# LinXueyuanStdio/LaTeX_OCR

Measured on NVIDIA H100. Metric: formula-images/sec (train step, 128x512 px, seq<=150), higher is better.
Workload: dtype bf16

## Files before the change

### latex_ocr_b200/csrc/lo_tc.cu

```cuda
#include <cuda.h>

#include <mutex>
#include <unordered_map>

#include "lo_common.cuh"
#include "lo_ptx.cuh"
#include "lo_wgmma.cuh"

namespace lo {

__device__ __forceinline__ void tma_load_2d(void* dst, const CUtensorMap* map, uint64_t* bar, int c0, int c1) {
  asm volatile("cp.async.bulk.tensor.2d.shared::cluster.global.mbarrier::complete_tx::bytes [%0], [%1, {%3, %4}], [%2];" ::"r"(
                   smem_u32(dst)),
               "l"(reinterpret_cast<uint64_t>(map)), "r"(smem_u32(bar)), "r"(c0), "r"(c1)
               : "memory");
}
__device__ __forceinline__ void tma_load_2d_hint(void* dst, const CUtensorMap* map, uint64_t* bar, int c0, int c1, uint64_t policy) {
  asm volatile(
      "cp.async.bulk.tensor.2d.shared::cluster.global.mbarrier::complete_tx::bytes.L2::cache_hint [%0], [%1, {%3, %4}], [%2], %5;" ::"r"(
          smem_u32(dst)),
      "l"(reinterpret_cast<uint64_t>(map)), "r"(smem_u32(bar)), "r"(c0), "r"(c1), "l"(policy)
      : "memory");
}
__device__ __forceinline__ void tma_load_3d(void* dst, const CUtensorMap* map, uint64_t* bar, int c0, int c1, int c2) {
// ... 62 lines not shown
  int64_t ldc;
  int out_f32, accumulate, relu;
  int kb_per_split, atomic;
  int w_evict_last;
  int half_w, half_h;
  long long* dbg;
  int lstm;
  const float* l_ptab; const int64_t* l_tok; int64_t l_tok_stride;
  const float* l_hh; int64_t l_hh_stride;
  const float* l_cprev; float* l_gates; float* l_c; float* l_h; bf16* l_hbf;
  float* l_hd; int64_t l_hd_stride; const float* l_dmask;
  int l_D, l_V;
};

constexpr int TC_BM = 128, TC_BK = 64;
constexpr int TC_CWARPS = 8;
constexpr int TC_THREADS = (TC_CWARPS + 2) * 32;

template <int NT, int STAGES>
struct TcSmem {
  static constexpr int A_BYTES = TC_BM * TC_BK * 2;
  static constexpr int B_BYTES = NT * TC_BK * 2;
  static constexpr int STAGE_BYTES = A_BYTES + B_BYTES;
  static constexpr int TOTAL = STAGES * STAGE_BYTES + 1024  + 256 ;
};

template <int NT>
__device__ __forceinline__ void tc_mma_kblock(float* acc, uint32_t sa, uint32_t sb, bool first) {
  const uint64_t da = make_kmajor_sw128_desc(sa), db = make_kmajor_sw128_desc(sb);
#pragma unroll
  for (int k = 0; k < TC_BK / 16; k++)
    Wgmma<NT, 0, 0>::mma(acc, da + (uint64_t)(2 * k), db + (uint64_t)(2 * k), (first && k == 0) ? 0u : 1u);
}

__device__ __forceinline__ void tc_store_pair(const TcParams& p, int64_t off, float f0, float f1, bool use_mask) {
  if (p.atomic) {
    float* o = reinterpret_cast<float*>(p.out) + off;
    atomicAdd(o, f0);
    atomicAdd(o + 1, f1);
  } else if (p.out_f32) {
    float2* o = reinterpret_cast<float2*>(reinterpret_cast<float*>(p.out) + off);
    if (p.accumulate) { const float2 old = *o; f0 += old.x; f1 += old.y; }
    if (p.relu) { f0 = fmaxf(f0, 0.f); f1 = fmaxf(f1, 0.f); }
    *o = make_float2(f0, f1);
  } else {
    uint32_t* o = reinterpret_cast<uint32_t*>(reinterpret_cast<bf16*>(p.out) + off);
    if (p.accumulate) { const uint32_t old = *o; f0 += __uint_as_float(old << 16); f1 += __uint_as_float(old & 0xffff0000u); }
    if (p.relu) { f0 = fmaxf(f0, 0.f); f1 = fmaxf(f1, 0.f); }
    if (use_mask) {
      const uint32_t w = *reinterpret_cast<const uint32_t*>(p.mask + off);
      if (!(__uint_as_float(w << 16) > 0.f)) f0 = 0.f;
      if (!(__uint_as_float(w & 0xffff0000u) > 0.f)) f1 = 0.f;
    }
    __nv_bfloat162 h = __floats2bfloat162_rn(f0, f1);
    *o = *reinterpret_cast<uint32_t*>(&h);
  }
}

template <int NT, int STAGES, int MC>
__global__ void __launch_bounds__(TC_THREADS, 1) tc_gemm_conv_kernel(const __grid_constant__ CUtensorMap mapA,
                                                                      const __grid_constant__ CUtensorMap mapB, TcParams p) {
  using SM = TcSmem<NT, STAGES>;
  extern __shared__ uint8_t smem_raw[];
  uint8_t* smem = reinterpret_cast<uint8_t*>((reinterpret_cast<uintptr_t>(smem_raw) + 1023) & ~(uintptr_t)1023);
  uint64_t* full_bar = reinterpret_cast<uint64_t*>(smem + STAGES * SM::STAGE_BYTES);
  uint64_t* empty_bar = full_bar + STAGES;
  __shared__ __align__(16) float s_bias[NT];

  const int warp = threadIdx.x >> 5, lane = threadIdx.x & 31;
  const int n0 = blockIdx.x * NT;
  const int mt = blockIdx.y;
  const int KB_all = p.K / TC_BK;
  const int kb0 = blockIdx.z * p.kb_per_split;
  const int KB = min(KB_all, kb0 + p.kb_per_split) - kb0;

  int img = 0, h0 = 0, w0 = 0, m0 = mt * TC_BM;
  if (p.conv) {
    const int per_img = p.tiles_w * p.tiles_h;
    img = mt / per_img;
    const int rem = mt % per_img;
    h0 = (rem / p.tiles_w) * p.BH;
    w0 = (rem % p.tiles_w) * p.BW;
  }

  const bool dbg = p.dbg && blockIdx.x == 0 && blockIdx.y == 0 && blockIdx.z == 0;
  if (dbg && threadIdx.x == 0) p.dbg[0] = clock64();
  if (warp == TC_CWARPS && lane == 0) {
    tma_prefetch_desc(&mapA);
    tma_prefetch_desc(&mapB);
    for (int s = 0; s < STAGES; s++) {
      mbar_init(full_bar + s, 2);
      mbar_init(empty_bar + s, MC ? 2 * TC_CWARPS : TC_CWARPS);
    }
    fence_barrier_init();
  }
  pdl_wait();
  pdl_trigger();
  if (MC) cluster_sync_all(); else __syncthreads();
  const uint32_t crank = MC ? cluster_ctarank() : 0;
  if (dbg && threadIdx.x == 0) p.dbg[1] = clock64();

  if (warp == TC_CWARPS) {
    if (lane == 0) {
      const int cpb = p.conv ? p.Cin / TC_BK : 1;
      for (int kb = 0; kb < KB; kb++) {
        const int s = kb % STAGES;
        const uint32_t ph = (kb / STAGES) & 1;
        mbar_wait(empty_bar + s, ph ^ 1);
        uint8_t* sa = smem + s * SM::STAGE_BYTES;
        mbar_expect_tx(full_bar + s, SM::A_BYTES);
        const int kg = kb0 + kb;
        if (MC) {
          uint8_t* sh = sa + crank * (SM::A_BYTES / 2);
          if (p.conv) {
            const int tap = kg / cpb, cb = kg % cpb;
            const int r = tap / 3, q = tap % 3;
            tma_load_4d_mc(sh, &mapA, full_bar + s, cb * TC_BK, w0 + (int)crank * p.half_w + q - p.pad,
                           h0 + (int)crank * p.half_h + r - p.pad, img, (uint16_t)3);
          } else {
            tma_load_2d_mc(sh, &mapA, full_bar + s, kg * TC_BK, m0 + (int)crank * (TC_BM / 2), (uint16_t)3);
          }
        } else if (p.conv) {
          const int tap = kg / cpb, cb = kg % cpb;
          const int r = tap / 3, q = tap % 3;
          tma_load_4d(sa, &mapA, full_bar + s, cb * TC_BK, w0 + q - p.pad, h0 + r - p.pad, img);
        } else {
          tma_load_2d(sa, &mapA, full_bar + s, kg * TC_BK, m0);
        }
        if (dbg && kb == 0) p.dbg[2] = clock64();
        if (dbg && kb < 40) p.dbg[64 + kb] = clock64();
      }
      if (dbg) p.dbg[3] = clock64();
    }
    __syncwarp();
  } else if (warp == TC_CWARPS + 1) {
    if (lane == 0) {
      const uint64_t polB = p.w_evict_last ? l2_policy_evict_last() : l2_policy_evict_normal();
      for (int kb = 0; kb < KB; kb++) {
        const int s = kb % STAGES;
        const uint32_t ph = (kb / STAGES) & 1;
        mbar_wait(empty_bar + s, ph ^ 1);
        uint8_t* sb = smem + s * SM::STAGE_BYTES + SM::A_BYTES;
        mbar_expect_tx(full_bar + s, SM::B_BYTES);
        tma_load_2d_hint(sb, &mapB, full_bar + s, (kb0 + kb) * TC_BK, n0, polB);
      }
    }
    __syncwarp();
  } else {
    const int wg = warp >> 2;
    for (int c = threadIdx.x; c < NT; c += TC_CWARPS * 32)
      s_bias[c] = (p.bias && blockIdx.z == 0 && n0 + c < p.N) ? __ldg(p.bias + n0 + c) : 0.f;
    asm volatile("bar.sync 1, 256;" ::: "memory");
    float acc[NT / 2];
    for (int kb = 0; kb < KB; kb++) {
      const int s = kb % STAGES;
      const uint32_t ph = (kb / STAGES) & 1;
      mbar_wait(full_bar + s, ph);
      if (dbg && threadIdx.x == 0 && kb == 0) p.dbg[4] = clock64();
      if (dbg && threadIdx.x == 0 && kb < 40) p.dbg[16 + kb] = clock64();
      const uint32_t sa = smem_u32(smem + s * SM::STAGE_BYTES);
      wgmma_fence();
      tc_mma_kblock<NT>(acc, sa + wg * (SM::A_BYTES / 2), sa + SM::A_BYTES, kb == 0);
      wgmma_commit();
      wgmma_wait0();
      wgmma_acc_fence<NT / 2>(acc);
      __syncwarp();
      if (lane == 0) {
        if (MC) { mbar_arrive_cta(empty_bar + s, 0); mbar_arrive_cta(empty_bar + s, 1); }
        else mbar_arrive(empty_bar + s);
      }
    }
    if (dbg && threadIdx.x == 0) p.dbg[5] = clock64();
    const int rbase = wg * 64 + (warp & 3) * 16 + (lane >> 2);
    const int cq = 2 * (lane & 3);
    if (p.lstm) {
      const int D = p.l_D;
#pragma unroll
      for (int h = 0; h < 2; h++) {
        const int b = m0 + rbase + 8 * h;
#pragma unroll
        for (int i = 0; i < NT / 8; i++) {
          const float a0 = acc[4 * i + 2 * h], a1 = acc[4 * i + 2 * h + 1];
          const float o0 = __shfl_xor_sync(0xffffffffu, a0, 1), o1 = __shfl_xor_sync(0xffffffffu, a1, 1);
          const int j = (n0 + 8 * i + cq) / 4;
          if ((lane & 1) || b >= p.M || j >= D) continue;
          int64_t tk = p.l_tok[(int64_t)b * p.l_tok_stride];
          tk = tk < 0 ? 0 : (tk >= p.l_V ? p.l_V - 1 : tk);
          const float* pt = p.l_ptab + tk * 4 * D;
          const float* hh = p.l_hh + (int64_t)b * p.l_hh_stride;
          const float pi = a0 + pt[j] + hh[j];
          const float pf = a1 + pt[D + j] + hh[D + j];
          const float pg = o0 + pt[2 * D + j] + hh[2 * D + j];
          const float po = o1 + pt[3 * D + j] + hh[3 * D + j];
          const float ig = sigmoidf_(pi), fg = sigmoidf_(pf), gg = tanhf(pg), og = sigmoidf_(po);
          const float cn = fg * p.l_cprev[(int64_t)b * D + j] + ig * gg;
          const float hn = og * tanhf(cn);
          float* gt = p.l_gates + (int64_t)b * 4 * D;
          gt[j] = ig; gt[D + j] = fg; gt[2 * D + j] = gg; gt[3 * D + j] = og;
          p.l_c[(int64_t)b * D + j] = cn;
          p.l_h[(int64_t)b * D + j] = hn;
          if (p.l_hbf) p.l_hbf[(int64_t)b * D + j] = __float2bfloat16_rn(hn);
          if (p.l_hd) p.l_hd[(int64_t)b * p.l_hd_stride + j] = p.l_dmask ? hn * p.l_dmask[(int64_t)b * p.l_hd_stride + j] : hn;
        }
      }
    } else {
      const bool use_mask = p.mask && !p.out_f32 && !p.atomic;
#pragma unroll
      for (int h = 0; h < 2; h++) {
        const int row = rbase + 8 * h;
        bool row_ok;
        int64_t row_off;
        if (p.conv) {
          const int hh = h0 + row / p.BW, ww = w0 + row % p.BW;
          row_ok = (hh < p.Ho) && (ww < p.Wo);
          row_off = (((int64_t)img * p.Ho + hh) * p.Wo + ww) * p.ldc;
        } else {
          row_ok = (m0 + row) < p.M;
          row_off = (int64_t)(m0 + row) * p.ldc;
        }
        if (!row_ok) continue;
#pragma unroll
        for (int i = 0; i < NT / 8; i++) {
          if (n0 + 8 * i >= p.N) continue;
          const int c = 8 * i + cq;
          tc_store_pair(p, row_off + n0 + c, acc[4 * i + 2 * h] + s_bias[c], acc[4 * i + 2 * h + 1] + s_bias[c + 1], use_mask);
        }
      }
    }
    if (dbg && threadIdx.x == 0) p.dbg[6] = clock64();
  }
  if (MC) cluster_sync_all();
  if (dbg && threadIdx.x == 0) p.dbg[7] = clock64();
}

template <int NT, int STAGES, int MT>
struct TcPSmem {
  static constexpr int A_BYTES = TC_BM * TC_BK * 2;
  static constexpr int B_BYTES = NT * TC_BK * 2;
  static constexpr int STAGE_BYTES = MT * A_BYTES + B_BYTES;
  static constexpr int TOTAL = STAGES * STAGE_BYTES + 1024  + 256  + 2 * NT * 4 ;
};

template <int NT, int STAGES, int MT>
__global__ void __launch_bounds__(TC_THREADS, 1) tc_conv_p_kernel(const __grid_constant__ CUtensorMap mapA,
                                                                 const __grid_constant__ CUtensorMap mapB, TcParams p, int ntiles_n,
                                                                 int total_tiles, int mtiles) {
  using SM = TcPSmem<NT, STAGES, MT>;
  static_assert(MT * NT <= 256, "accumulator registers");
  extern __shared__ uint8_t smem_raw[];
  uint8_t* smem = reinterpret_cast<uint8_t*>((reinterpret_cast<uintptr_t>(smem_raw) + 1023) & ~(uintptr_t)1023);
  uint64_t* full_bar = reinterpret_cast<uint64_t*>(smem + STAGES * SM::STAGE_BYTES);
  uint64_t* empty_bar = full_bar + STAGES;
  float* s_bias = reinterpret_cast<float*>(smem + STAGES * SM::STAGE_BYTES + 256);

  const int warp = threadIdx.x >> 5, lane = threadIdx.x & 31;
  const int KB = p.K / TC_BK;
  const int cpb = p.Cin / TC_BK;
  const int per_img = p.tiles_w * p.tiles_h;

  if (warp == TC_CWARPS && lane == 0) {
    tma_prefetch_desc(&mapA);
    tma_prefetch_desc(&mapB);
    for (int s = 0; s < STAGES; s++) {
      mbar_init(full_bar + s, 2);
      mbar_init(empty_bar + s, TC_CWARPS);
    }
    fence_barrier_init();
  }
  pdl_wait();
  pdl_trigger();
  __syncthreads();

  if (warp == TC_CWARPS) {
    if (lane == 0) {
      uint32_t it = 0;
      for (int tile = blockIdx.x; tile < total_tiles; tile += gridDim.x) {
        const int mt0 = (tile / ntiles_n) * MT;
        const int nsub = min(MT, mtiles - mt0);
        int img[MT], h0[MT], w0[MT];
#pragma unroll
        for (int j = 0; j < MT; j++) {
          const int mt = min(mt0 + j, mtiles - 1);
          img[j] = mt / per_img;
          const int rem = mt % per_img;
          h0[j] = (rem / p.tiles_w) * p.BH;
          w0[j] = (rem % p.tiles_w) * p.BW;
        }
        for (int kb = 0; kb < KB; kb++, it++) {
          const int s = it % STAGES;
          const uint32_t ph = (it / STAGES) & 1;
          mbar_wait(empty_bar + s, ph ^ 1);
          mbar_expect_tx(full_bar + s, (uint32_t)nsub * SM::A_BYTES);
          const int tap = kb / cpb, cb = kb % cpb;
          const int r = tap / 3, q = tap % 3;
#pragma unroll
          for (int j = 0; j < MT; j++)
            if (j < nsub)
              tma_load_4d(smem + s * SM::STAGE_BYTES + j * SM::A_BYTES, &mapA, full_bar + s, cb * TC_BK, w0[j] + q - p.pad,
                          h0[j] + r - p.pad, img[j]);
        }
      }
    }
    __syncwarp();
  } else if (warp == TC_CWARPS + 1) {
    if (lane == 0) {
      const uint64_t polB = l2_policy_evict_last();
      uint32_t it = 0;
      for (int tile = blockIdx.x; tile < total_tiles; tile += gridDim.x) {
        const int n0 = (tile % ntiles_n) * NT;
        for (int kb = 0; kb < KB; kb++, it++) {
          const int s = it % STAGES;
          const uint32_t ph = (it / STAGES) & 1;
          mbar_wait(empty_bar + s, ph ^ 1);
          mbar_expect_tx(full_bar + s, SM::B_BYTES);
          tma_load_2d_hint(smem + s * SM::STAGE_BYTES + MT * SM::A_BYTES, &mapB, full_bar + s, kb * TC_BK, n0, polB);
        }
      }
    }
    __syncwarp();
  } else {
    const int wg = warp >> 2;
    const int rbase = wg * 64 + (warp & 3) * 16 + (lane >> 2);
    const int cq = 2 * (lane & 3);
    const bool use_mask = p.mask != nullptr;
    uint32_t it = 0, lt = 0;
    for (int tile = blockIdx.x; tile < total_tiles; tile += gridDim.x, lt++) {
      const int n0 = (tile % ntiles_n) * NT;
      const int mt0 = (tile / ntiles_n) * MT;
      const int nsub = min(MT, mtiles - mt0);
      float* sb = s_bias + (lt & 1) * NT;
      for (int c = threadIdx.x; c < NT; c += TC_CWARPS * 32) sb[c] = (p.bias && n0 + c < p.N) ? __ldg(p.bias + n0 + c) : 0.f;
      asm volatile("bar.sync 1, 256;" ::: "memory");
      float acc[MT][NT / 2];
      for (int kb = 0; kb < KB; kb++, it++) {
        const int s = it % STAGES;
        const uint32_t ph = (it / STAGES) & 1;
        mbar_wait(full_bar + s, ph);
        const uint32_t sa = smem_u32(smem + s * SM::STAGE_BYTES);
        wgmma_fence();
#pragma unroll
        for (int j = 0; j < MT; j++)
          tc_mma_kblock<NT>(acc[j], sa + j * SM::A_BYTES + wg * (SM::A_BYTES / 2), sa + MT * SM::A_BYTES, kb == 0);
        wgmma_commit();
        wgmma_wait0();
#pragma unroll
        for (int j = 0; j < MT; j++) wgmma_acc_fence<NT / 2>(acc[j]);
        __syncwarp();
        if (lane == 0) mbar_arrive(empty_bar + s);
      }
#pragma unroll
      for (int j = 0; j < MT; j++) {
        if (j >= nsub) continue;
        const int mt = mt0 + j;
        const int img = mt / per_img, rem = mt % per_img;
#pragma unroll
        for (int h = 0; h < 2; h++) {
          const int row = rbase + 8 * h;
          const int hh = (rem / p.tiles_w) * p.BH + row / p.BW, ww = (rem % p.tiles_w) * p.BW + row % p.BW;
          if (hh >= p.Ho || ww >= p.Wo) continue;
          const int64_t row_off = (((int64_t)img * p.Ho + hh) * p.Wo + ww) * p.ldc;
#pragma unroll
          for (int i = 0; i < NT / 8; i++) {
            if (n0 + 8 * i >= p.N) continue;
            const int c = 8 * i + cq;
            float f0 = acc[j][4 * i + 2 * h] + sb[c], f1 = acc[j][4 * i + 2 * h + 1] + sb[c + 1];
            if (p.relu) { f0 = fmaxf(f0, 0.f); f1 = fmaxf(f1, 0.f); }
            if (use_mask) {
              const uint32_t w = *reinterpret_cast<const uint32_t*>(p.mask + row_off + n0 + c);
              if (!(__uint_as_float(w << 16) > 0.f)) f0 = 0.f;
              if (!(__uint_as_float(w & 0xffff0000u) > 0.f)) f1 = 0.f;
            }
            __nv_bfloat162 hv = __floats2bfloat162_rn(f0, f1);
            *reinterpret_cast<__nv_bfloat162*>(reinterpret_cast<bf16*>(p.out) + row_off + n0 + c) = hv;
          }
        }
      }
    }
  }
}

__device__ __forceinline__ uint64_t make_mnmajor_sw128_desc(uint32_t saddr, uint32_t lbo_bytes) {
  uint64_t d = 0;
  d |= (uint64_t)((saddr & 0x3FFFF) >> 4);
  d |= (uint64_t)((lbo_bytes >> 4) & 0x3FFF) << 16;
  d |= (uint64_t)(1024 >> 4) << 32;
  d |= (uint64_t)1 << 62;
  return d;
}

struct WgParams {
  int Cin, Cout, Ho, Wo, pad;
  int BW, BH, tiles_w, tiles_h, kstages, per_split, ci_tiles;
  float* dw;
  int plain;
  int64_t ldc;
  int64_t batch_c;
  int ordered;
};

template <int NT, int STAGES>
__global__ void __launch_bounds__(TC_THREADS, 1) tc_wgrad_kernel(const __grid_constant__ CUtensorMap mapDY,
                                                                  const __grid_constant__ CUtensorMap mapX, WgParams p) {
  constexpr int BOX = 128 * 64 * 2;
  constexpr int A_BYTES = 2 * BOX, B_BYTES = (NT / 64) * BOX, STAGE_BYTES = A_BYTES + B_BYTES;
  extern __shared__ uint8_t smem_raw[];
  uint8_t* smem = reinterpret_cast<uint8_t*>((reinterpret_cast<uintptr_t>(smem_raw) + 1023) & ~(uintptr_t)1023);
  uint64_t* full_bar = reinterpret_cast<uint64_t*>(smem + STAGES * STAGE_BYTES);
  uint64_t* empty_bar = full_bar + STAGES;
  const int warp = threadIdx.x >> 5, lane = threadIdx.x & 31;
  const int co0 = (blockIdx.x / p.ci_tiles) * 128, ci0 = (blockIdx.x % p.ci_tiles) * NT;
  const int tap = p.plain == 2 ? 0 : blockIdx.y, r = tap / 3, q = tap % 3;
  const int bz = p.plain == 2 ? blockIdx.y : 0;
  const int ks0 = blockIdx.z * p.per_split;
  const int ks1 = min(p.kstages, ks0 + p.per_split);
  const int KS = ks1 - ks0;
  if (warp == TC_CWARPS && lane == 0) {
    tma_prefetch_desc(&mapDY);
    tma_prefetch_desc(&mapX);
    for (int s = 0; s < STAGES; s++) { mbar_init(full_bar + s, 2); mbar_init(empty_bar + s, TC_CWARPS); }
    fence_barrier_init();
  }
  __syncthreads();
  float acc[NT / 2];
  if (warp == TC_CWARPS) {
    if (lane == 0) {
      const int per_img = p.tiles_w * p.tiles_h;
      for (int i = 0; i < KS; i++) {
        const int s = i % STAGES;
        const uint32_t ph = (i / STAGES) & 1;
        mbar_wait(empty_bar + s, ph ^ 1);
        const int ks = ks0 + i;
        const int img = ks / per_img, rem = ks % per_img;
        const int h0 = (rem / p.tiles_w) * p.BH, w0 = (rem % p.tiles_w) * p.BW;
        uint8_t* sa = smem + s * STAGE_BYTES;
        mbar_expect_tx(full_bar + s, A_BYTES);
        if (p.plain == 2) {
          tma_load_3d(sa, &mapDY, full_bar + s, co0, ks * 128, bz);
          tma_load_3d(sa + BOX, &mapDY, full_bar + s, co0 + 64, ks * 128, bz);
        } else if (p.plain) {
          tma_load_2d(sa, &mapDY, full_bar + s, co0, ks * 128);
          tma_load_2d(sa + BOX, &mapDY, full_bar + s, co0 + 64, ks * 128);
        } else {
          tma_load_4d(sa, &mapDY, full_bar + s, co0, w0, h0, img);
          tma_load_4d(sa + BOX, &mapDY, full_bar + s, co0 + 64, w0, h0, img);
        }
      }
    }
    __syncwarp();
  } else if (warp == TC_CWARPS + 1) {
    if (lane == 0) {
      const int per_img = p.tiles_w * p.tiles_h;
      for (int i = 0; i < KS; i++) {
        const int s = i % STAGES;
        const uint32_t ph = (i / STAGES) & 1;
        mbar_wait(empty_bar + s, ph ^ 1);
        const int ks = ks0 + i;
        const int img = ks / per_img, rem = ks % per_img;
        const int h0 = (rem / p.tiles_w) * p.BH, w0 = (rem % p.tiles_w) * p.BW;
        uint8_t* sb = smem + s * STAGE_BYTES + A_BYTES;
        mbar_expect_tx(full_bar + s, B_BYTES);
        if (p.plain == 2) {
#pragma unroll
          for (int j = 0; j < NT / 64; j++) tma_load_3d(sb + j * BOX, &mapX, full_bar + s, ci0 + 64 * j, ks * 128, bz);
        } else if (p.plain) {
#pragma unroll
          for (int j = 0; j < NT / 64; j++) tma_load_2d(sb + j * BOX, &mapX, full_bar + s, ci0 + 64 * j, ks * 128);
        } else {
#pragma unroll
          for (int j = 0; j < NT / 64; j++)
            tma_load_4d(sb + j * BOX, &mapX, full_bar + s, ci0 + 64 * j, w0 + q - p.pad, h0 + r - p.pad, img);
        }
      }
    }
    __syncwarp();
  } else {
    const int wg = warp >> 2;
#pragma unroll
    for (int i = 0; i < NT / 2; i++) acc[i] = 0.f;
    for (int i = 0; i < KS; i++) {
      const int s = i % STAGES;
      const uint32_t ph = (i / STAGES) & 1;
      mbar_wait(full_bar + s, ph);
      const uint32_t sa = smem_u32(smem + s * STAGE_BYTES) + wg * BOX;
      const uint32_t sb = smem_u32(smem + s * STAGE_BYTES) + A_BYTES;
      wgmma_fence();
#pragma unroll
      for (int k = 0; k < 8; k++)
        Wgmma<NT, 1, 1>::mma(acc, make_mnmajor_sw128_desc(sa + k * 2048, BOX), make_mnmajor_sw128_desc(sb + k * 2048, BOX), 1u);
      wgmma_commit();
      wgmma_wait0();
      wgmma_acc_fence<NT / 2>(acc);
      __syncwarp();
      if (lane == 0) mbar_arrive(empty_bar + s);
    }
  }
  if (p.ordered && gridDim.z > 1) {
    float* part = reinterpret_cast<float*>(smem);
    if (warp < TC_CWARPS) {
      asm volatile("bar.sync 1, 256;" ::: "memory");
#pragma unroll
      for (int i = 0; i < NT / 2; i++) part[i * 256 + threadIdx.x] = acc[i];
    }
    cl_sync();
    if (cl_rank() == 0 && warp < TC_CWARPS) {
#pragma unroll
      for (int i = 0; i < NT / 2; i += 16) cl_sum_n<16>(part + i * 256 + threadIdx.x, 256, acc + i);
    }
    cl_sync();
    if (cl_rank() != 0) return;
  }
  if (warp < TC_CWARPS) {
    const int wg = warp >> 2, cq = 2 * (lane & 3);
#pragma unroll
    for (int h = 0; h < 2; h++) {
      const int co = co0 + wg * 64 + (warp & 3) * 16 + (lane >> 2) + 8 * h;
      if (co >= p.Cout) continue;
      float* orow = p.plain ? p.dw + (int64_t)bz * p.batch_c + (int64_t)co * p.ldc : p.dw + ((int64_t)co * 9 + tap) * p.Cin;
#pragma unroll
      for (int i = 0; i < NT / 8; i++) {
        const int ci = ci0 + 8 * i + cq;
        if (ci < p.Cin) atomicAdd(orow + ci, acc[4 * i + 2 * h]);
        if (ci + 1 < p.Cin) atomicAdd(orow + ci + 1, acc[4 * i + 2 * h + 1]);
      }
    }
  }
}

typedef CUresult (*PFN_tmapEncodeTiled)(CUtensorMap*, CUtensorMapDataType, cuuint32_t, void*, const cuuint64_t*, const cuuint64_t*,
                                        const cuuint32_t*, const cuuint32_t*, CUtensorMapInterleave, CUtensorMapSwizzle,
                                        CUtensorMapL2promotion, CUtensorMapFloatOOBfill);
static PFN_tmapEncodeTiled g_encode = nullptr;
static int g_tc_state = -1;

bool tc_available() {
  if (g_tc_state >= 0) return g_tc_state == 1;
  g_tc_state = 0;
  int dev = 0, major = 0;
  if (cudaGetDevice(&dev) != cudaSuccess) return false;
  if (cudaDeviceGetAttribute(&major, cudaDevAttrComputeCapabilityMajor, dev) != cudaSuccess || major != 9) return false;
  void* fn = nullptr;
  cudaDriverEntryPointQueryResult qres;
  if (cudaGetDriverEntryPoint("cuTensorMapEncodeTiled", &fn, cudaEnableDefault, &qres) != cudaSuccess || fn == nullptr ||
      qres != cudaDriverEntryPointSuccess)
    return false;
  g_encode = (PFN_tmapEncodeTiled)fn;
  g_tc_state = 1;
  return true;
}

struct MapKey {
  const void* base; int rank; cuuint64_t dims[4]; cuuint64_t str[3]; cuuint32_t box[4];
  bool operator==(const MapKey& o) const { return memcmp(this, &o, sizeof(MapKey)) == 0; }
};
struct MapKeyHash {
  size_t operator()(const MapKey& k) const {
    const uint64_t* w = reinterpret_cast<const uint64_t*>(&k);
    uint64_t h = 1469598103934665603ull;
    for (size_t i = 0; i < sizeof(MapKey) / 8; i++) { h ^= w[i]; h *= 1099511628211ull; }
    return (size_t)h;
  }
};
static std::unordered_map<MapKey, CUtensorMap, MapKeyHash> g_map_cache;
static std::mutex g_map_mutex;

static int make_map(CUtensorMap* m, const void* base, int rank, const cuuint64_t* dims, const cuuint64_t* strides_bytes,
                    const cuuint32_t* box) {
  MapKey key;
  memset(&key, 0, sizeof(key));
  key.base = base; key.rank = rank;
  for (int i = 0; i < rank; i++) { key.dims[i] = dims[i]; key.box[i] = box[i]; }
  for (int i = 0; i + 1 < rank; i++) key.str[i] = strides_bytes[i];
  {
    std::lock_guard<std::mutex> lk(g_map_mutex);
    auto it = g_map_cache.find(key);
    if (it != g_map_cache.end()) { *m = it->second; return LO_OK; }
  }
  cuuint32_t estr[4] = {1, 1, 1, 1};
  CUresult r = g_encode(m, CU_TENSOR_MAP_DATA_TYPE_BFLOAT16, (cuuint32_t)rank, const_cast<void*>(base), dims, strides_bytes, box, estr,
                        CU_TENSOR_MAP_INTERLEAVE_NONE, CU_TENSOR_MAP_SWIZZLE_128B, CU_TENSOR_MAP_L2_PROMOTION_L2_256B,
                        CU_TENSOR_MAP_FLOAT_OOB_FILL_NONE);
  if (r != CUDA_SUCCESS) return fail(LO_ECUDA, "%s: cuTensorMapEncodeTiled failed (%ld)", "tc", (long)r);
  std::lock_guard<std::mutex> lk(g_map_mutex);
  if (g_map_cache.size() > 20000) g_map_cache.clear();
  g_map_cache.emplace(key, *m);
  return LO_OK;
}

int g_opt_conv_mc = 1;
long long* g_tc_dbg = nullptr;
int g_opt_skinny8 = 1;

template <int NT, int STAGES, int MC>
static int launch_tc(const CUtensorMap& mA, const CUtensorMap& mB, const TcParams& p, int mtiles, int splits, cudaStream_t st) {
  using SM = TcSmem<NT, STAGES>;
  static bool attr_set = false;
  if (!attr_set) {
    LO_CUDA(cudaFuncSetAttribute(tc_gemm_conv_kernel<NT, STAGES, MC>, cudaFuncAttributeMaxDynamicSharedMemorySize, SM::TOTAL));
    attr_set = true;
  }
  dim3 grid(cdiv(p.N, NT), mtiles, splits);
  cudaLaunchConfig_t cfg{};
  cfg.gridDim = grid;
  cfg.blockDim = dim3(TC_THREADS);
  cfg.dynamicSmemBytes = SM::TOTAL;
  cfg.stream = st;
  cudaLaunchAttribute attr[2];
  int n = 0;
  if (g_opt_pdl) {
    attr[n].id = cudaLaunchAttributeProgrammaticStreamSerialization;
    attr[n].val.programmaticStreamSerializationAllowed = 1;
    n++;
  }
  if (MC) {
    attr[n].id = cudaLaunchAttributeClusterDimension;
    attr[n].val.clusterDim.x = 2;
    attr[n].val.clusterDim.y = 1;
    attr[n].val.clusterDim.z = 1;
    n++;
  }
  cfg.attrs = attr;
  cfg.numAttrs = n;
  LO_CUDA(cudaLaunchKernelEx(&cfg, tc_gemm_conv_kernel<NT, STAGES, MC>, mA, mB, p));
  LO_LAUNCH_OK();
  return LO_OK;
}

static int launch_tc_any(const CUtensorMap& mA, const CUtensorMap& mB, TcParams& p, int mtiles, int splits, int nt, cudaStream_t st,
                         int mc = 0) {
  const int KB = p.K / TC_BK;
  if (splits < 1) splits = 1;
  if (splits > KB) splits = KB;
  p.kb_per_split = cdiv(KB, splits);
  splits = cdiv(KB, p.kb_per_split);
  p.atomic = splits > 1 ? 1 : p.atomic;
  if (nt == 64 && mtiles == 1 && p.kb_per_split > 4 && g_opt_skinny8) return launch_tc<64, 8, 0>(mA, mB, p, mtiles, splits, st);
  if (nt == 64) return launch_tc<64, 4, 0>(mA, mB, p, mtiles, splits, st);
  if (mc) return launch_tc<128, 3, 1>(mA, mB, p, mtiles, splits, st);
  return launch_tc<128, 3, 0>(mA, mB, p, mtiles, splits, st);
}

static TcLstmEpi g_lstm_epi;
static bool g_lstm_epi_on = false;

int tc_gemm_nt_ex(const bf16* A, int64_t lda, const bf16* W, int64_t ldw, void* C, int dtC, int64_t ldc, int M, int N, int K,
                  const float* bias, int accumulate, int relu, int splits, int atomic_acc, int small_n_tile, cudaStream_t st) {
  if (!tc_available()) return fail(LO_ENOTSUP, "%s: needs an sm_90 device", __func__);
  LO_CHECK_ARG(K % 64 == 0 && lda % 8 == 0 && ldw % 8 == 0 && ldc % 8 == 0 && ldc >= (N + 7) / 8 * 8, "K%64, ld%8, ldc >= roundup8(N)");
  LO_CHECK_ARG(((uintptr_t)A & 15) == 0 && ((uintptr_t)W & 15) == 0 && ((uintptr_t)C & 15) == 0, "16-byte alignment");
  CUtensorMap mA, mB;
  const int NT = (N <= 64 || small_n_tile) ? 64 : 128;
  const int mc = (g_opt_conv_mc && NT == 128 && cdiv(N, 128) % 2 == 0 && splits <= 1 && !atomic_acc) ? 1 : 0;
  {
    cuuint64_t dims[2] = {(cuuint64_t)K, (cuuint64_t)M};
    cuuint64_t str[1] = {(cuuint64_t)lda * 2};
    cuuint32_t box[2] = {64, (cuuint32_t)(mc ? 64 : 128)};
    LO_TRY(make_map(&mA, A, 2, dims, str, box));
  }
  {
    cuuint64_t dims[2] = {(cuuint64_t)K, (cuuint64_t)N};
    cuuint64_t str[1] = {(cuuint64_t)ldw * 2};
    cuuint32_t box[2] = {64, (cuuint32_t)NT};
    LO_TRY(make_map(&mB, W, 2, dims, str, box));
  }
  LO_CHECK_ARG(!(splits > 1 || atomic_acc) || (dtC == LO_F32 && !relu), "split-K needs fp32 output without ReLU");
  TcParams p{};
  p.M = M; p.N = N; p.K = K; p.conv = 0;
  p.bias = bias; p.mask = nullptr; p.out = C; p.ldc = ldc;
  p.out_f32 = (dtC == LO_F32); p.accumulate = accumulate; p.relu = relu; p.atomic = atomic_acc;
  p.w_evict_last = (M <= 128) ? 1 : 0;
  p.dbg = g_tc_dbg;
  if (g_lstm_epi_on) {
    const TcLstmEpi& e = g_lstm_epi;
    p.lstm = 1;
    p.l_ptab = e.ptab; p.l_tok = e.tok; p.l_tok_stride = e.tok_stride; p.l_hh = e.hh; p.l_hh_stride = e.hh_stride;
    p.l_cprev = e.c_prev; p.l_gates = e.gates; p.l_c = e.c_out; p.l_h = e.h_out; p.l_hbf = e.h_bf;
    p.l_hd = e.hd; p.l_hd_stride = e.hd_stride; p.l_dmask = e.dmask; p.l_D = e.D; p.l_V = e.V;
  }
  return launch_tc_any(mA, mB, p, cdiv(M, TC_BM), splits, NT, st, mc);
}

int tc_gemm_nt_lstm(const bf16* A, int64_t lda, const bf16* Wil, int64_t ldw, int M, int D, int K, const TcLstmEpi& e, cudaStream_t st) {
  g_lstm_epi = e;
  g_lstm_epi_on = true;
  const int r = tc_gemm_nt_ex(A, lda, Wil, ldw, e.gates , LO_F32, 4 * D, M, 4 * D, K, nullptr, 0, 0, 1, 0, 1, st);
  g_lstm_epi_on = false;
  return r;
}

int tc_gemm_nt(const bf16* A, int64_t lda, const bf16* W, int64_t ldw, void* C, int dtC, int64_t ldc, int M, int N, int K,
               const float* bias, int accumulate, int relu, cudaStream_t st) {
  return tc_gemm_nt_ex(A, lda, W, ldw, C, dtC, ldc, M, N, K, bias, accumulate, relu, 1, 0, 0, st);
}

int g_opt_wgrad256 = 0;
int g_opt_conv_persist = 1;

int g_opt_conv_mt2 = 1;

template <int NT, int STAGES, int MT>
static int launch_conv_p(const CUtensorMap& mA, const CUtensorMap& mB, const TcParams& p, int mtiles, cudaStream_t st) {
  using SM = TcPSmem<NT, STAGES, MT>;
  static bool attr_set = false;
  static int n_sm = 0;
  if (!attr_set) {
    LO_CUDA(cudaFuncSetAttribute(tc_conv_p_kernel<NT, STAGES, MT>, cudaFuncAttributeMaxDynamicSharedMemorySize, SM::TOTAL));
    int dev = 0;
    LO_CUDA(cudaGetDevice(&dev));
    LO_CUDA(cudaDeviceGetAttribute(&n_sm, cudaDevAttrMultiProcessorCount, dev));
    attr_set = true;
  }
  const int ntn = cdiv(p.N, NT);
  const int total = cdiv(mtiles, MT) * ntn;
  const int grid = total < n_sm ? total : n_sm;
  LO_CUDA(launch_pdl(tc_conv_p_kernel<NT, STAGES, MT>, dim3(grid), dim3(TC_THREADS), (size_t)SM::TOTAL, st, mA, mB, p, ntn, total, mtiles));
  LO_LAUNCH_OK();
  return LO_OK;
}

int tc_conv3x3(const bf16* x, const bf16* w, const float* bias, const bf16* mask, bf16* y, int N, int H, int W, int Cin, int Cout,
               int pad, int relu, cudaStream_t st) {
  if (!tc_available()) return fail(LO_ENOTSUP, "%s: needs an sm_90 device", __func__);
  LO_CHECK_ARG(Cin % 64 == 0 && Cout % 8 == 0, "Cin%64==0, Cout%8==0");
  const int Ho = H + 2 * pad - 2, Wo = W + 2 * pad - 2;
  int BW = 128;
  while (BW > 8 && BW / 2 >= Wo) BW /= 2;
  const int BH = 128 / BW;
  if (g_opt_conv_persist) {
    const int NTp = Cout % 256 == 0 ? 256 : (Cout > 64 ? 128 : 64);
    CUtensorMap mA, mB;
    {
      cuuint64_t dims[4] = {(cuuint64_t)Cin, (cuuint64_t)W, (cuuint64_t)H, (cuuint64_t)N};
      cuuint64_t str[3] = {(cuuint64_t)Cin * 2, (cuuint64_t)W * Cin * 2, (cuuint64_t)H * W * Cin * 2};
      cuuint32_t box[4] = {64, (cuuint32_t)BW, (cuuint32_t)BH, 1};
      LO_TRY(make_map(&mA, x, 4, dims, str, box));
    }
    {
      cuuint64_t dims[2] = {(cuuint64_t)9 * Cin, (cuuint64_t)Cout};
      cuuint64_t str[1] = {(cuuint64_t)9 * Cin * 2};
      cuuint32_t box[2] = {64, (cuuint32_t)NTp};
      LO_TRY(make_map(&mB, w, 2, dims, str, box));
    }
    TcParams p{};
    p.M = N * Ho * Wo; p.N = Cout; p.K = 9 * Cin; p.conv = 1;
    p.Ho = Ho; p.Wo = Wo; p.Cin = Cin; p.pad = pad;
    p.BW = BW; p.BH = BH; p.tiles_w = cdiv(Wo, BW); p.tiles_h = cdiv(Ho, BH);
    p.bias = bias; p.mask = mask; p.out = y; p.ldc = Cout; p.relu = relu;
    const int mtiles = N * p.tiles_w * p.tiles_h;
    if (NTp == 256) return launch_conv_p<256, 4, 1>(mA, mB, p, mtiles, st);
    if (NTp == 128) return g_opt_conv_mt2 ? launch_conv_p<128, 4, 2>(mA, mB, p, mtiles, st) : launch_conv_p<128, 6, 1>(mA, mB, p, mtiles, st);
    return g_opt_conv_mt2 ? launch_conv_p<64, 4, 2>(mA, mB, p, mtiles, st) : launch_conv_p<64, 8, 1>(mA, mB, p, mtiles, st);
  }
  CUtensorMap mA, mB;
  const int NT = Cout <= 64 ? 64 : 128;
  const int mc = (g_opt_conv_mc && NT == 128 && cdiv(Cout, 128) % 2 == 0) ? 1 : 0;
  const int hbw = mc ? (BH >= 2 ? BW : BW / 2) : BW, hbh = mc ? (BH >= 2 ? BH / 2 : 1) : BH;
  {
    cuuint64_t dims[4] = {(cuuint64_t)Cin, (cuuint64_t)W, (cuuint64_t)H, (cuuint64_t)N};
    cuuint64_t str[3] = {(cuuint64_t)Cin * 2, (cuuint64_t)W * Cin * 2, (cuuint64_t)H * W * Cin * 2};
    cuuint32_t box[4] = {64, (cuuint32_t)hbw, (cuuint32_t)hbh, 1};
    LO_TRY(make_map(&mA, x, 4, dims, str, box));
  }
  {
    cuuint64_t dims[2] = {(cuuint64_t)9 * Cin, (cuuint64_t)Cout};
    cuuint64_t str[1] = {(cuuint64_t)9 * Cin * 2};
    cuuint32_t box[2] = {64, (cuuint32_t)NT};
    LO_TRY(make_map(&mB, w, 2, dims, str, box));
  }
  TcParams p{};
  p.M = N * Ho * Wo; p.N = Cout; p.K = 9 * Cin; p.conv = 1;
  p.Ho = Ho; p.Wo = Wo; p.Cin = Cin; p.pad = pad;
  p.BW = BW; p.BH = BH; p.tiles_w = cdiv(Wo, BW); p.tiles_h = cdiv(Ho, BH);
  p.bias = bias; p.mask = mask; p.out = y; p.ldc = Cout;
  p.out_f32 = 0; p.accumulate = 0; p.relu = relu;
  p.dbg = g_tc_dbg;
  p.half_w = (mc && BH < 2) ? BW / 2 : 0;
  p.half_h = (mc && BH >= 2) ? BH / 2 : 0;
  const int mtiles = N * p.tiles_w * p.tiles_h;
  LO_CHECK_ARG(mtiles <= 65535, "too many M tiles for grid.y");
  return launch_tc_any(mA, mB, p, mtiles, 1, NT, st, mc);
}


template <int NT, int STAGES>
static int launch_wgrad(const CUtensorMap& mDY, const CUtensorMap& mX, const WgParams& p, dim3 grid, cudaStream_t st) {
  constexpr int TOTAL = STAGES * (2 + NT / 64) * 16384 + 1024 + 256;
  static bool attr_set = false;
  if (!attr_set) {
    LO_CUDA(cudaFuncSetAttribute(tc_wgrad_kernel<NT, STAGES>, cudaFuncAttributeMaxDynamicSharedMemorySize, TOTAL));
    attr_set = true;
  }
  if (p.ordered)
    LO_CUDA(launch_cluster(tc_wgrad_kernel<NT, STAGES>, grid, dim3(TC_THREADS), (size_t)TOTAL, st, dim3(1, 1, grid.z), false, mDY, mX, p));
  else
    tc_wgrad_kernel<NT, STAGES><<<grid, TC_THREADS, TOTAL, st>>>(mDY, mX, p);
  LO_LAUNCH_OK();
  return LO_OK;
}

int tc_conv3x3_wgrad(const bf16* x, const bf16* dy, float* dw, int N, int H, int W, int Cin, int Cout, int pad, cudaStream_t st) {
  if (!tc_available()) return fail(LO_ENOTSUP, "%s: needs an sm_90 device", __func__);
  LO_CHECK_ARG(Cin % 64 == 0 && Cout % 128 == 0, "Cin%64==0, Cout%128==0");
  const int Ho = H + 2 * pad - 2, Wo = W + 2 * pad - 2;
  int BW = 128;
  while (BW > 8 && BW / 2 >= Wo) BW /= 2;
  const int BH = 128 / BW;
  CUtensorMap mDY, mX;
  {
    cuuint64_t dims[4] = {(cuuint64_t)Cout, (cuuint64_t)Wo, (cuuint64_t)Ho, (cuuint64_t)N};
    cuuint64_t str[3] = {(cuuint64_t)Cout * 2, (cuuint64_t)Wo * Cout * 2, (cuuint64_t)Ho * Wo * Cout * 2};
    cuuint32_t box[4] = {64, (cuuint32_t)BW, (cuuint32_t)BH, 1};
    LO_TRY(make_map(&mDY, dy, 4, dims, str, box));
  }
  {
    cuuint64_t dims[4] = {(cuuint64_t)Cin, (cuuint64_t)W, (cuuint64_t)H, (cuuint64_t)N};
    cuuint64_t str[3] = {(cuuint64_t)Cin * 2, (cuuint64_t)W * Cin * 2, (cuuint64_t)H * W * Cin * 2};
    cuuint32_t box[4] = {64, (cuuint32_t)BW, (cuuint32_t)BH, 1};
    LO_TRY(make_map(&mX, x, 4, dims, str, box));
  }
  WgParams p{};
  p.Cin = Cin; p.Cout = Cout; p.Ho = Ho; p.Wo = Wo; p.pad = pad;
  p.BW = BW; p.BH = BH; p.tiles_w = cdiv(Wo, BW); p.tiles_h = cdiv(Ho, BH);
  p.kstages = N * p.tiles_w * p.tiles_h;
  p.dw = dw;
  const int NT = (g_opt_wgrad256 && Cin % 256 == 0) ? 256 : (Cin >= 128 ? 128 : 64);
  p.ci_tiles = Cin / NT;
  const int tiles = (Cout / 128) * p.ci_tiles * 9;
  int splits = cdiv(NT == 256 ? LO_NUM_SMS : LO_NUM_SMS * 2, tiles);
  if (g_opt_det && splits > 8) splits = 8;
  if (splits > p.kstages) splits = p.kstages;
  if (splits < 1) splits = 1;
  p.per_split = cdiv(p.kstages, splits);
  splits = cdiv(p.kstages, p.per_split);
  p.ordered = g_opt_det && splits > 1;
  dim3 grid((Cout / 128) * p.ci_tiles, 9, splits);
  if (NT == 256) return launch_wgrad<256, 2>(mDY, mX, p, grid, st);
  if (NT == 128) return launch_wgrad<128, 3>(mDY, mX, p, grid, st);
  return launch_wgrad<64, 4>(mDY, mX, p, grid, st);
}

int tc_gemm_tn(const bf16* A, int64_t lda, const bf16* B, int64_t ldb, float* C, int64_t ldc, int M, int N, int K, cudaStream_t st) {
  if (!tc_available()) return fail(LO_ENOTSUP, "%s: needs an sm_90 device", __func__);
  LO_CHECK_ARG(lda % 8 == 0 && ldb % 8 == 0, "lda%8, ldb%8");
  LO_CHECK_ARG(((uintptr_t)A & 15) == 0 && ((uintptr_t)B & 15) == 0, "16-byte alignment");
  CUtensorMap mA, mB;
  {
    cuuint64_t dims[2] = {(cuuint64_t)M, (cuuint64_t)K};
    cuuint64_t str[1] = {(cuuint64_t)lda * 2};
    cuuint32_t box[2] = {64, 128};
    LO_TRY(make_map(&mA, A, 2, dims, str, box));
  }
  {
    cuuint64_t dims[2] = {(cuuint64_t)N, (cuuint64_t)K};
    cuuint64_t str[1] = {(cuuint64_t)ldb * 2};
    cuuint32_t box[2] = {64, 128};
    LO_TRY(make_map(&mB, B, 2, dims, str, box));
  }
  WgParams p{};
  p.plain = 1; p.Cout = M; p.Cin = N; p.dw = C; p.ldc = ldc;
  p.tiles_w = p.tiles_h = 1; p.BW = 128; p.BH = 1;
  p.kstages = cdiv(K, 128);
  const int NT = N > 64 ? 128 : 64;
  p.ci_tiles = cdiv(N, NT);
  const int mt = cdiv(M, 128);
  const int tiles = mt * p.ci_tiles;
  int splits = cdiv(LO_NUM_SMS * 2, tiles);
  if (g_opt_det && splits > 8) splits = 8;
  if (splits > p.kstages) splits = p.kstages;
  if (splits < 1) splits = 1;
  p.per_split = cdiv(p.kstages, splits);
  splits = cdiv(p.kstages, p.per_split);
  p.ordered = g_opt_det && splits > 1;
  dim3 grid(mt * p.ci_tiles, 1, splits);
  if (NT == 128) return launch_wgrad<128, 3>(mA, mB, p, grid, st);
  return launch_wgrad<64, 4>(mA, mB, p, grid, st);
}

int tc_gemm_tn_batched(const bf16* A, int64_t sAk, int64_t sAb, const bf16* B, int64_t sBk, int64_t sBb, float* C, int64_t ldc,
                       int64_t sCb, int M, int N, int K, int batch, cudaStream_t st) {
  if (!tc_available()) return fail(LO_ENOTSUP, "%s: needs an sm_90 device", __func__);
  LO_CHECK_ARG(sAk % 8 == 0 && sAb % 8 == 0 && sBk % 8 == 0 && sBb % 8 == 0, "strides must be multiples of 8 elements");
  LO_CHECK_ARG(((uintptr_t)A & 15) == 0 && ((uintptr_t)B & 15) == 0 && batch >= 1 && batch <= 65535, "alignment / batch");
  CUtensorMap mA, mB;
  {
    cuuint64_t dims[3] = {(cuuint64_t)M, (cuuint64_t)K, (cuuint64_t)batch};
    cuuint64_t str[2] = {(cuuint64_t)sAk * 2, (cuuint64_t)sAb * 2};
    cuuint32_t box[3] = {64, 128, 1};
    LO_TRY(make_map(&mA, A, 3, dims, str, box));
  }
  {
    cuuint64_t dims[3] = {(cuuint64_t)N, (cuuint64_t)K, (cuuint64_t)batch};
    cuuint64_t str[2] = {(cuuint64_t)sBk * 2, (cuuint64_t)sBb * 2};
    cuuint32_t box[3] = {64, 128, 1};
    LO_TRY(make_map(&mB, B, 3, dims, str, box));
  }
  WgParams p{};
  p.plain = 2; p.Cout = M; p.Cin = N; p.dw = C; p.ldc = ldc; p.batch_c = sCb;
  p.tiles_w = p.tiles_h = 1; p.BW = 128; p.BH = 1;
  p.kstages = cdiv(K, 128);
  p.per_split = p.kstages;
  const int NT = N > 64 ? 128 : 64;
  p.ci_tiles = cdiv(N, NT);
  dim3 grid(cdiv(M, 128) * p.ci_tiles, batch, 1);
  if (NT == 128) return launch_wgrad<128, 3>(mA, mB, p, grid, st);
  return launch_wgrad<64, 4>(mA, mB, p, grid, st);
}

}
```

### latex_ocr_b200/csrc/lo_wgmma.cuh

```cuda
#pragma once
#include <stdint.h>

namespace lo {

__device__ __forceinline__ void wgmma_fence() { asm volatile("wgmma.fence.sync.aligned;" ::: "memory"); }
__device__ __forceinline__ void wgmma_commit() { asm volatile("wgmma.commit_group.sync.aligned;" ::: "memory"); }
__device__ __forceinline__ void wgmma_wait0() { asm volatile("wgmma.wait_group.sync.aligned 0;" ::: "memory"); }
template <int NREG>
__device__ __forceinline__ void wgmma_acc_fence(float* d) {
#pragma unroll
  for (int i = 0; i < NREG; i++) asm volatile("" : "+f"(d[i])::"memory");
}

template <int N, int TA, int TB>
struct Wgmma;
template <int TA, int TB>
struct Wgmma<64, TA, TB> {
  __device__ __forceinline__ static void mma(float* d, uint64_t da, uint64_t db, uint32_t scale_d) {
    asm volatile(
        "{\n"
        ".reg .pred p;\n"
        "setp.ne.b32 p, %34, 0;\n"
        "wgmma.mma_async.sync.aligned.m64n64k16.f32.bf16.bf16 {"
        "%0, %1, %2, %3, %4, %5, %6, %7, %8, %9, %10, %11, %12, %13, %14, %15, "
        "%16, %17, %18, %19, %20, %21, %22, %23, %24, %25, %26, %27, %28, %29, %30, %31"
        "}, %32, %33, p, 1, 1, %35, %36;\n"
        "}\n"
        : "+f"(d[0]), "+f"(d[1]), "+f"(d[2]), "+f"(d[3]), "+f"(d[4]), "+f"(d[5]), "+f"(d[6]), "+f"(d[7]), "+f"(d[8]),
        "+f"(d[9]), "+f"(d[10]), "+f"(d[11]), "+f"(d[12]), "+f"(d[13]), "+f"(d[14]), "+f"(d[15]), "+f"(d[16]),
        "+f"(d[17]), "+f"(d[18]), "+f"(d[19]), "+f"(d[20]), "+f"(d[21]), "+f"(d[22]), "+f"(d[23]), "+f"(d[24]),
        "+f"(d[25]), "+f"(d[26]), "+f"(d[27]), "+f"(d[28]), "+f"(d[29]), "+f"(d[30]), "+f"(d[31])
        : "l"(da), "l"(db), "r"(scale_d), "n"(TA), "n"(TB));
  }
};

template <int TA, int TB>
struct Wgmma<128, TA, TB> {
  __device__ __forceinline__ static void mma(float* d, uint64_t da, uint64_t db, uint32_t scale_d) {
    asm volatile(
        "{\n"
        ".reg .pred p;\n"
        "setp.ne.b32 p, %66, 0;\n"
        "wgmma.mma_async.sync.aligned.m64n128k16.f32.bf16.bf16 {"
        "%0, %1, %2, %3, %4, %5, %6, %7, %8, %9, %10, %11, %12, %13, %14, %15, "
        "%16, %17, %18, %19, %20, %21, %22, %23, %24, %25, %26, %27, %28, %29, %30, %31, "
        "%32, %33, %34, %35, %36, %37, %38, %39, %40, %41, %42, %43, %44, %45, %46, %47, "
        "%48, %49, %50, %51, %52, %53, %54, %55, %56, %57, %58, %59, %60, %61, %62, %63"
        "}, %64, %65, p, 1, 1, %67, %68;\n"
        "}\n"
        : "+f"(d[0]), "+f"(d[1]), "+f"(d[2]), "+f"(d[3]), "+f"(d[4]), "+f"(d[5]), "+f"(d[6]), "+f"(d[7]), "+f"(d[8]),
        "+f"(d[9]), "+f"(d[10]), "+f"(d[11]), "+f"(d[12]), "+f"(d[13]), "+f"(d[14]), "+f"(d[15]), "+f"(d[16]),
        "+f"(d[17]), "+f"(d[18]), "+f"(d[19]), "+f"(d[20]), "+f"(d[21]), "+f"(d[22]), "+f"(d[23]), "+f"(d[24]),
        "+f"(d[25]), "+f"(d[26]), "+f"(d[27]), "+f"(d[28]), "+f"(d[29]), "+f"(d[30]), "+f"(d[31]), "+f"(d[32]),
        "+f"(d[33]), "+f"(d[34]), "+f"(d[35]), "+f"(d[36]), "+f"(d[37]), "+f"(d[38]), "+f"(d[39]), "+f"(d[40]),
        "+f"(d[41]), "+f"(d[42]), "+f"(d[43]), "+f"(d[44]), "+f"(d[45]), "+f"(d[46]), "+f"(d[47]), "+f"(d[48]),
        "+f"(d[49]), "+f"(d[50]), "+f"(d[51]), "+f"(d[52]), "+f"(d[53]), "+f"(d[54]), "+f"(d[55]), "+f"(d[56]),
        "+f"(d[57]), "+f"(d[58]), "+f"(d[59]), "+f"(d[60]), "+f"(d[61]), "+f"(d[62]), "+f"(d[63])
        : "l"(da), "l"(db), "r"(scale_d), "n"(TA), "n"(TB));
  }
};

template <int TA, int TB>
struct Wgmma<256, TA, TB> {
  __device__ __forceinline__ static void mma(float* d, uint64_t da, uint64_t db, uint32_t scale_d) {
    asm volatile(
        "{\n"
        ".reg .pred p;\n"
        "setp.ne.b32 p, %130, 0;\n"
        "wgmma.mma_async.sync.aligned.m64n256k16.f32.bf16.bf16 {"
        "%0, %1, %2, %3, %4, %5, %6, %7, %8, %9, %10, %11, %12, %13, %14, %15, "
        "%16, %17, %18, %19, %20, %21, %22, %23, %24, %25, %26, %27, %28, %29, %30, %31, "
        "%32, %33, %34, %35, %36, %37, %38, %39, %40, %41, %42, %43, %44, %45, %46, %47, "
        "%48, %49, %50, %51, %52, %53, %54, %55, %56, %57, %58, %59, %60, %61, %62, %63, "
        "%64, %65, %66, %67, %68, %69, %70, %71, %72, %73, %74, %75, %76, %77, %78, %79, "
        "%80, %81, %82, %83, %84, %85, %86, %87, %88, %89, %90, %91, %92, %93, %94, %95, "
        "%96, %97, %98, %99, %100, %101, %102, %103, %104, %105, %106, %107, %108, %109, %110, %111, "
        "%112, %113, %114, %115, %116, %117, %118, %119, %120, %121, %122, %123, %124, %125, %126, %127"
        "}, %128, %129, p, 1, 1, %131, %132;\n"
        "}\n"
        : "+f"(d[0]), "+f"(d[1]), "+f"(d[2]), "+f"(d[3]), "+f"(d[4]), "+f"(d[5]), "+f"(d[6]), "+f"(d[7]), "+f"(d[8]),
        "+f"(d[9]), "+f"(d[10]), "+f"(d[11]), "+f"(d[12]), "+f"(d[13]), "+f"(d[14]), "+f"(d[15]), "+f"(d[16]),
        "+f"(d[17]), "+f"(d[18]), "+f"(d[19]), "+f"(d[20]), "+f"(d[21]), "+f"(d[22]), "+f"(d[23]), "+f"(d[24]),
        "+f"(d[25]), "+f"(d[26]), "+f"(d[27]), "+f"(d[28]), "+f"(d[29]), "+f"(d[30]), "+f"(d[31]), "+f"(d[32]),
        "+f"(d[33]), "+f"(d[34]), "+f"(d[35]), "+f"(d[36]), "+f"(d[37]), "+f"(d[38]), "+f"(d[39]), "+f"(d[40]),
        "+f"(d[41]), "+f"(d[42]), "+f"(d[43]), "+f"(d[44]), "+f"(d[45]), "+f"(d[46]), "+f"(d[47]), "+f"(d[48]),
        "+f"(d[49]), "+f"(d[50]), "+f"(d[51]), "+f"(d[52]), "+f"(d[53]), "+f"(d[54]), "+f"(d[55]), "+f"(d[56]),
        "+f"(d[57]), "+f"(d[58]), "+f"(d[59]), "+f"(d[60]), "+f"(d[61]), "+f"(d[62]), "+f"(d[63]), "+f"(d[64]),
        "+f"(d[65]), "+f"(d[66]), "+f"(d[67]), "+f"(d[68]), "+f"(d[69]), "+f"(d[70]), "+f"(d[71]), "+f"(d[72]),
        "+f"(d[73]), "+f"(d[74]), "+f"(d[75]), "+f"(d[76]), "+f"(d[77]), "+f"(d[78]), "+f"(d[79]), "+f"(d[80]),
        "+f"(d[81]), "+f"(d[82]), "+f"(d[83]), "+f"(d[84]), "+f"(d[85]), "+f"(d[86]), "+f"(d[87]), "+f"(d[88]),
        "+f"(d[89]), "+f"(d[90]), "+f"(d[91]), "+f"(d[92]), "+f"(d[93]), "+f"(d[94]), "+f"(d[95]), "+f"(d[96]),
        "+f"(d[97]), "+f"(d[98]), "+f"(d[99]), "+f"(d[100]), "+f"(d[101]), "+f"(d[102]), "+f"(d[103]), "+f"(d[104]),
        "+f"(d[105]), "+f"(d[106]), "+f"(d[107]), "+f"(d[108]), "+f"(d[109]), "+f"(d[110]), "+f"(d[111]), "+f"(d[112]),
        "+f"(d[113]), "+f"(d[114]), "+f"(d[115]), "+f"(d[116]), "+f"(d[117]), "+f"(d[118]), "+f"(d[119]), "+f"(d[120]),
        "+f"(d[121]), "+f"(d[122]), "+f"(d[123]), "+f"(d[124]), "+f"(d[125]), "+f"(d[126]), "+f"(d[127])
        : "l"(da), "l"(db), "r"(scale_d), "n"(TA), "n"(TB));
  }
};

}
```

Baseline: 2076.

## Overlap wgmma groups across k-blocks and pick wgrad split-K by occupancy cost model

The GEMM and conv consumer loops now wait with wait_group 1 instead of 0, so the next k-block's wgmma can issue while the previous one completes. The smem stage is released one iteration later, with a final drain after the loop. Separately, the non-deterministic weight-gradient launch chooses split-K count from a cost model that uses measured occupancy (SM count times blocks per SM) instead of a fixed heuristic. The risks are a stage being held longer, which reduces effective pipeline depth, and accumulator hazards if the fences are insufficient.

Result: no change. 2104 (median of 6 runs) (+1.3%).

```diff
diff --git a/latex_ocr_b200/csrc/lo_tc.cu b/latex_ocr_b200/csrc/lo_tc.cu
--- a/latex_ocr_b200/csrc/lo_tc.cu
+++ b/latex_ocr_b200/csrc/lo_tc.cu
@@ -238,6 +238,13 @@
       s_bias[c] = (p.bias && blockIdx.z == 0 && n0 + c < p.N) ? __ldg(p.bias + n0 + c) : 0.f;
     asm volatile("bar.sync 1, 256;" ::: "memory");
     float acc[NT / 2];
+    auto release = [&](int s) {
+      __syncwarp();
+      if (lane == 0) {
+        if (MC) { mbar_arrive_cta(empty_bar + s, 0); mbar_arrive_cta(empty_bar + s, 1); }
+        else mbar_arrive(empty_bar + s);
+      }
+    };
     for (int kb = 0; kb < KB; kb++) {
       const int s = kb % STAGES;
       const uint32_t ph = (kb / STAGES) & 1;
@@ -248,14 +255,13 @@
       wgmma_fence();
       tc_mma_kblock<NT>(acc, sa + wg * (SM::A_BYTES / 2), sa + SM::A_BYTES, kb == 0);
       wgmma_commit();
-      wgmma_wait0();
+      wgmma_wait<1>();
       wgmma_acc_fence<NT / 2>(acc);
-      __syncwarp();
-      if (lane == 0) {
-        if (MC) { mbar_arrive_cta(empty_bar + s, 0); mbar_arrive_cta(empty_bar + s, 1); }
-        else mbar_arrive(empty_bar + s);
-      }
-    }
+      if (kb > 0) release((kb - 1) % STAGES);
+    }
+    wgmma_wait<0>();
+    wgmma_acc_fence<NT / 2>(acc);
+    if (KB > 0) release((KB - 1) % STAGES);
     if (dbg && threadIdx.x == 0) p.dbg[5] = clock64();
     const int rbase = wg * 64 + (warp & 3) * 16 + (lane >> 2);
     const int cq = 2 * (lane & 3);
@@ -428,12 +434,17 @@
         for (int j = 0; j < MT; j++)
           tc_mma_kblock<NT>(acc[j], sa + j * SM::A_BYTES + wg * (SM::A_BYTES / 2), sa + MT * SM::A_BYTES, kb == 0);
         wgmma_commit();
-        wgmma_wait0();
+        wgmma_wait<1>();
 #pragma unroll
         for (int j = 0; j < MT; j++) wgmma_acc_fence<NT / 2>(acc[j]);
         __syncwarp();
-        if (lane == 0) mbar_arrive(empty_bar + s);
-      }
+        if (kb > 0 && lane == 0) mbar_arrive(empty_bar + (it - 1) % STAGES);
+      }
+      wgmma_wait<0>();
+#pragma unroll
+      for (int j = 0; j < MT; j++) wgmma_acc_fence<NT / 2>(acc[j]);
+      __syncwarp();
+      if (lane == 0) mbar_arrive(empty_bar + (it - 1) % STAGES);
 #pragma unroll
       for (int j = 0; j < MT; j++) {
         if (j >= nsub) continue;
@@ -574,7 +585,7 @@
       for (int k = 0; k < 8; k++)
         Wgmma<NT, 1, 1>::mma(acc, make_mnmajor_sw128_desc(sa + k * 2048, BOX), make_mnmajor_sw128_desc(sb + k * 2048, BOX), 1u);
       wgmma_commit();
-      wgmma_wait0();
+      wgmma_wait<0>();
       wgmma_acc_fence<NT / 2>(acc);
       __syncwarp();
       if (lane == 0) mbar_arrive(empty_bar + s);
@@ -868,13 +879,45 @@
 
 
 template <int NT, int STAGES>
+struct WgSmem {
+  static constexpr int TOTAL = STAGES * (2 + NT / 64) * 16384 + 1024 + 256;
+};
+
+template <int NT, int STAGES>
+static int wgrad_slots() {
+  static int slots = 0;
+  if (!slots) {
+    int dev = 0, n_sm = 0, per_sm = 0;
+    if (cudaFuncSetAttribute(tc_wgrad_kernel<NT, STAGES>, cudaFuncAttributeMaxDynamicSharedMemorySize, WgSmem<NT, STAGES>::TOTAL) !=
+            cudaSuccess ||
+        cudaGetDevice(&dev) != cudaSuccess || cudaDeviceGetAttribute(&n_sm, cudaDevAttrMultiProcessorCount, dev) != cudaSuccess ||
+        cudaOccupancyMaxActiveBlocksPerMultiprocessor(&per_sm, tc_wgrad_kernel<NT, STAGES>, TC_THREADS, WgSmem<NT, STAGES>::TOTAL) !=
+            cudaSuccess)
+      return 0;
+    slots = n_sm * per_sm;
+  }
+  return slots;
+}
+
+static int wgrad_splits(int tiles, int kstages, int slots) {
+  constexpr int kFill = 4, kAtomic = 4;
+  if (slots < 1) return 1;
+  int best = 1;
+  double best_cost = 1e300;
+  for (int s = 1; s <= kstages && (int64_t)tiles * s <= 16 * (int64_t)slots; s++) {
+    const int per = cdiv(kstages, s);
+    if (cdiv(kstages, per) != s) continue;
+    const int64_t ctas = (int64_t)tiles * s, rounds = (ctas + slots - 1) / slots;
+    const double cost = (double)rounds * (per + kFill) + (double)kAtomic * ctas / slots;
+    if (cost < best_cost) { best_cost = cost; best = s; }
+  }
+  return best;
+}
+
+template <int NT, int STAGES>
 static int launch_wgrad(const CUtensorMap& mDY, const CUtensorMap& mX, const WgParams& p, dim3 grid, cudaStream_t st) {
-  constexpr int TOTAL = STAGES * (2 + NT / 64) * 16384 + 1024 + 256;
-  static bool attr_set = false;
-  if (!attr_set) {
-    LO_CUDA(cudaFuncSetAttribute(tc_wgrad_kernel<NT, STAGES>, cudaFuncAttributeMaxDynamicSharedMemorySize, TOTAL));
-    attr_set = true;
-  }
+  constexpr int TOTAL = WgSmem<NT, STAGES>::TOTAL;
+  if (wgrad_slots<NT, STAGES>() == 0) return fail(LO_ECUDA, "%s: cannot size the weight-gradient grid", __func__);
   if (p.ordered)
     LO_CUDA(launch_cluster(tc_wgrad_kernel<NT, STAGES>, grid, dim3(TC_THREADS), (size_t)TOTAL, st, dim3(1, 1, grid.z), false, mDY, mX, p));
   else
@@ -911,8 +954,13 @@
   const int NT = (g_opt_wgrad256 && Cin % 256 == 0) ? 256 : (Cin >= 128 ? 128 : 64);
   p.ci_tiles = Cin / NT;
   const int tiles = (Cout / 128) * p.ci_tiles * 9;
-  int splits = cdiv(NT == 256 ? LO_NUM_SMS : LO_NUM_SMS * 2, tiles);
-  if (g_opt_det && splits > 8) splits = 8;
+  int splits;
+  if (g_opt_det) {
+    splits = cdiv(NT == 256 ? LO_NUM_SMS : LO_NUM_SMS * 2, tiles);
+    if (splits > 8) splits = 8;
+  } else {
+    splits = wgrad_splits(tiles, p.kstages, NT == 256 ? wgrad_slots<256, 2>() : NT == 128 ? wgrad_slots<128, 3>() : wgrad_slots<64, 4>());
+  }
   if (splits > p.kstages) splits = p.kstages;
   if (splits < 1) splits = 1;
   p.per_split = cdiv(p.kstages, splits);
@@ -949,8 +997,13 @@
   p.ci_tiles = cdiv(N, NT);
   const int mt = cdiv(M, 128);
   const int tiles = mt * p.ci_tiles;
-  int splits = cdiv(LO_NUM_SMS * 2, tiles);
-  if (g_opt_det && splits > 8) splits = 8;
+  int splits;
+  if (g_opt_det) {
+    splits = cdiv(LO_NUM_SMS * 2, tiles);
+    if (splits > 8) splits = 8;
+  } else {
+    splits = wgrad_splits(tiles, p.kstages, NT == 128 ? wgrad_slots<128, 3>() : wgrad_slots<64, 4>());
+  }
   if (splits > p.kstages) splits = p.kstages;
   if (splits < 1) splits = 1;
   p.per_split = cdiv(p.kstages, splits);
diff --git a/latex_ocr_b200/csrc/lo_wgmma.cuh b/latex_ocr_b200/csrc/lo_wgmma.cuh
--- a/latex_ocr_b200/csrc/lo_wgmma.cuh
+++ b/latex_ocr_b200/csrc/lo_wgmma.cuh
@@ -5,7 +5,8 @@
 
 __device__ __forceinline__ void wgmma_fence() { asm volatile("wgmma.fence.sync.aligned;" ::: "memory"); }
 __device__ __forceinline__ void wgmma_commit() { asm volatile("wgmma.commit_group.sync.aligned;" ::: "memory"); }
-__device__ __forceinline__ void wgmma_wait0() { asm volatile("wgmma.wait_group.sync.aligned 0;" ::: "memory"); }
+template <int N>
+__device__ __forceinline__ void wgmma_wait() { asm volatile("wgmma.wait_group.sync.aligned %0;" ::"n"(N) : "memory"); }
 template <int NREG>
 __device__ __forceinline__ void wgmma_acc_fence(float* d) {
 #pragma unroll
```
